# Human-Augment-Analytics/vectordb-retrieval

Measured on AMD Instinct MI355X. Metric: QPS @ recall@10 (SIFT1M-shaped, 10k-query batch, k=10), higher is better.
Workload: dtype i8 MFMA scan (i32 accumulate) + exact integer / f64 refine

## Files before the change

vectordb-retrieval_amd/csrc/common.hpp:

```cpp
#pragma once
#include <hip/hip_runtime.h>
#include <hip/hip_fp16.h>
#include <stdint.h>

#include <stdexcept>
#include <string>

namespace vdb {

constexpr int kTileRows = 32;
constexpr int kSpanRows = 512;
constexpr int kBinRows = 256;
constexpr int kTilesPerSpan = 16;
constexpr int kTileRows16 = 16;
constexpr int kSpanRows16 = 1024;
constexpr int kTilesPerSpan16 = 64;
constexpr int kIvfTilesPerSpan = 8;
constexpr int kIvfSpanRows = kIvfTilesPerSpan * kTileRows;
constexpr int kStageTiles = 4;
constexpr int kMaxKSteps = 8;
constexpr float kPadBias = 1.0e38f;

constexpr int kStatShards = 32;
constexpr int kStatStride = 16;
__device__ __forceinline__ void stat_add(unsigned long long *counters, long long q, int idx, unsigned long long v) {
    atomicAdd(&counters[(size_t)(q & (kStatShards - 1)) * kStatStride + idx], v);
}
constexpr size_t kSmallBytes = 64 + (size_t)kStatShards * kStatStride * 8;
constexpr size_t kInfoOffset = 16;

struct IndexStats {
    unsigned absmax_bits;
    unsigned maxnorm2_bits;
    int nonfinite;
    int not_integer;
    int not_fp16_exact;
    int not_u8;
    int not_s8;
    int pad[1];
};

struct QueryBatchInfo {
    unsigned absmax_bits;
    int not_integer;
    int not_fp16_exact;
    int nonfinite;
    float sq;
    float cs;
    float bscale;
    int force_fallback;
    int not_u8, not_s8;
    int i8_mode;
    unsigned done_blocks;
};
static_assert(sizeof(QueryBatchInfo) + 16 <= 64, "QueryBatchInfo must fit the first 64 bytes of ws.small");

__host__ __device__ inline int group_rows_of(int i8_mode) { return (i8_mode & 4) ? 8 : 4; }
__host__ __device__ inline int cand_row_offset(unsigned packed_bits, int i8_mode) {
    return (int)(packed_bits & 0x3Fu) * group_rows_of(i8_mode);
}
constexpr int kI8Offset = 1 << 24;
constexpr int kI8PadBias = 30000000;
constexpr unsigned kI8Inf = 0x7f800000u;

struct Range {
    int64_t row0;
    int32_t count;
    int32_t pad;
};

__host__ __device__ inline uint64_t sortable_u64(double v) {
    uint64_t u = *reinterpret_cast<uint64_t *>(&v);
    return (u & 0x8000000000000000ull) ? ~u : (u | 0x8000000000000000ull);
}
__host__ __device__ inline double unsortable_f64(uint64_t k) {
    uint64_t u = (k & 0x8000000000000000ull) ? (k & 0x7fffffffffffffffull) : ~k;
    return *reinterpret_cast<double *>(&u);
}
__host__ __device__ inline unsigned sortable_u32(float v) {
    unsigned u = *reinterpret_cast<unsigned *>(&v);
    return (u & 0x80000000u) ? ~u : (u | 0x80000000u);
}
__host__ __device__ inline float unsortable_f32(unsigned k) {
    unsigned u = (k & 0x80000000u) ? (k & 0x7fffffffu) : ~k;
    return *reinterpret_cast<float *>(&u);
}

struct Error : public std::runtime_error {
    int code;
    Error(int c, const std::string &m) : std::runtime_error(m), code(c) {}
};

#define VDB_HIP(expr)                                                                              \
    do {                                                                                           \
        hipError_t e__ = (expr);                                                                   \
        if (e__ != hipSuccess)                                                                     \
            throw ::vdb::Error(3, std::string(#expr) + " failed: " + hipGetErrorString(e__));      \
    } while (0)

}
```

vectordb-retrieval_amd/csrc/refine.hpp:

```cpp
#pragma once
#include "common.hpp"
#include "topk.hpp"

namespace vdb {

struct Sq8Rows {
    const unsigned char *codes = nullptr;
    const int32_t *list = nullptr;
    const float *cent = nullptr;
    const float *vmin = nullptr;
    const float *vdiff = nullptr;
};

__device__ __forceinline__ float sq8_decode(unsigned code, float c, float vmin, float vdiff) {
    return c + (vmin + (((float)code + 0.5f) / 255.0f) * vdiff);
}

struct PqRows {
    const unsigned char *codes = nullptr;
    const float *cb = nullptr;
    int M = 0, dsub = 0;
};

struct RefineCommon {
// ... 80 lines not shown
    const unsigned *cw = reinterpret_cast<const unsigned *>(s.codes + (size_t)row * D4);
    const float4 *cv = reinterpret_cast<const float4 *>(s.cent + (size_t)s.list[row] * D4);
    const float4 *mv = reinterpret_cast<const float4 *>(s.vmin);
    const float4 *dv = reinterpret_cast<const float4 *>(s.vdiff);
    const float4 *qv = reinterpret_cast<const float4 *>(q);
    double acc = 0.0;
#pragma unroll 4
    for (int i = 0; i < D4 / 4; ++i) {
        const unsigned w = cw[i];
        const float4 c = cv[i], m = mv[i], d = dv[i], b = qv[i];
        const double x0 = (double)sq8_decode(w & 0xffu, c.x, m.x, d.x);
        const double x1 = (double)sq8_decode((w >> 8) & 0xffu, c.y, m.y, d.y);
        const double x2 = (double)sq8_decode((w >> 16) & 0xffu, c.z, m.z, d.z);
        const double x3 = (double)sq8_decode(w >> 24, c.w, m.w, d.w);
        if (metric == 0) {
            double t;
            t = x0 - (double)b.x; acc = fma(t, t, acc);
            t = x1 - (double)b.y; acc = fma(t, t, acc);
            t = x2 - (double)b.z; acc = fma(t, t, acc);
            t = x3 - (double)b.w; acc = fma(t, t, acc);
        } else {
            acc = fma((double)b.x, x0, acc);
            acc = fma((double)b.y, x1, acc);
            acc = fma((double)b.z, x2, acc);
            acc = fma((double)b.w, x3, acc);
        }
    }
    return sortable_u64(metric == 0 ? acc : -acc);
}

__device__ __forceinline__ uint64_t pq_key(const PqRows &p, int64_t row, const float *__restrict__ q, int D4, int metric) {
    const unsigned char *cr = p.codes + (size_t)row * p.M;
    double acc = 0.0;
    int d = 0;
    for (int m = 0; m < p.M; ++m) {
        const float *cv = p.cb + ((size_t)m * 256 + cr[m]) * p.dsub;
        for (int j = 0; j < p.dsub; ++j, ++d) {
            const double x = (double)cv[j];
            if (metric == 0) {
                const double t = x - (double)q[d];
                acc = fma(t, t, acc);
            } else {
                acc = fma((double)q[d], x, acc);
            }
        }
    }
    for (; d < D4; ++d) {
        if (metric == 0) {
            const double t = 0.0 - (double)q[d];
            acc = fma(t, t, acc);
        } else {
            acc = fma((double)q[d], 0.0, acc);
        }
    }
    return sortable_u64(metric == 0 ? acc : -acc);
}

template <int U = 16>
__device__ __forceinline__ uint64_t row_key(const RefineCommon &c, int64_t row, const float *__restrict__ q) {
    if (c.X) return exact_key<U>(c.X + (size_t)row * c.D4, q, c.D4, c.metric);
    if (c.sq8.codes) return sq8_key(c.sq8, row, q, c.D4, c.metric);
    if (c.pq.codes) return pq_key(c.pq, row, q, c.D4, c.metric);
    return exact_key_i8<U>(c.X8 + (size_t)row * c.x8_pitch, c.cx, q, c.D4, c.metric);
}

template <int QB>
__device__ __forceinline__ void exact_keys(const float *__restrict__ x, const float *const (&q)[QB], int D4, int metric,
                                           uint64_t (&out)[QB]) {
    const float4 *xv = reinterpret_cast<const float4 *>(x);
    double acc[QB];
#pragma unroll
    for (int j = 0; j < QB; ++j) acc[j] = 0.0;
#pragma unroll 4
    for (int i = 0; i < D4 / 4; ++i) {
        const float4 a = xv[i];
#pragma unroll
        for (int j = 0; j < QB; ++j) {
            const float4 b = reinterpret_cast<const float4 *>(q[j])[i];
            if (metric == 0) {
                double t;
                t = (double)a.x - (double)b.x; acc[j] = fma(t, t, acc[j]);
                t = (double)a.y - (double)b.y; acc[j] = fma(t, t, acc[j]);
                t = (double)a.z - (double)b.z; acc[j] = fma(t, t, acc[j]);
                t = (double)a.w - (double)b.w; acc[j] = fma(t, t, acc[j]);
            } else {
                acc[j] = fma((double)b.x, (double)a.x, acc[j]);
                acc[j] = fma((double)b.y, (double)a.y, acc[j]);
                acc[j] = fma((double)b.z, (double)a.z, acc[j]);
                acc[j] = fma((double)b.w, (double)a.w, acc[j]);
            }
        }
    }
#pragma unroll
    for (int j = 0; j < QB; ++j) out[j] = sortable_u64(metric == 0 ? acc[j] : -acc[j]);
}

template <int KPL, int U = 16>
__device__ __forceinline__ void scan_rows(WaveTopK<KPL> &tk, const RefineCommon &c, const float *qptr, int64_t row0,
                                          int64_t row1) {
    const int lane = threadIdx.x & 63;
    if (row1 > c.N) row1 = c.N;
    for (int64_t base = row0; base < row1; base += 64) {
        const int64_t row = base + lane;
        const bool valid = row < row1;
        uint64_t key = ~0ull;
        if (valid) key = row_key<U>(c, row, qptr);
        tk.offer(key, c.idmap ? (valid ? c.idmap[row] : -1) : c.id_base + row, valid);
    }
}

template <int KPL>
__device__ __forceinline__ void write_topk(const WaveTopK<KPL> &tk, int metric, float *D, int64_t *I, double *pk,
                                           int64_t *pi) {
    const int lane = threadIdx.x & 63;
#pragma unroll
    for (int e = 0; e < KPL; ++e) {
        const int s = e * 64 + lane;
        if (s < tk.k) {
            const bool have = s < tk.n;
            const double kv = have ? unsortable_f64(tk.key[e]) : __builtin_inf();
            if (D) {
                float d;
                if (have)
                    d = (float)(metric == 0 ? kv : -kv);
                else
                    d = (metric == 0) ? 3.402823466e+38f : -3.402823466e+38f;
                D[s] = d;
                I[s] = have ? tk.id[e] : -1;
            } else {
                pk[s] = kv;
                pi[s] = have ? tk.id[e] : -1;
            }
        }
    }
}

struct RefineListArgs {
    RefineCommon c;
    int64_t nq;
    const int32_t *cand_rows;
    const int32_t *rescan_rows;
    const int32_t *counts;
    const int32_t *fallback;
    int cand_cap;
    int rescan_cap;
    float *D;
    int64_t *I;
    double *pkeys;
    int64_t *pids;
    int group_shift = -1;
    int f16_shift = 2;
};

template <int KPL, int W>
__device__ __forceinline__ void refine_list_dot8(const RefineListArgs &a, int64_t q, int ncand, int nres, int gshift,
                                                 WaveTopK<KPL> &tk) {
    const int lane = threadIdx.x & 63;
    const RefineCommon &c = a.c;
    const int mode = c.info->i8_mode;
    const int cq = (mode & 3) == 1 ? 127 : -1;
    int qb[W];
    const int *q8 = reinterpret_cast<const int *>(c.Q8 + (size_t)q * c.x8_pitch);
#pragma unroll
    for (int w = 0; w < W; ++w) qb[w] = __builtin_amdgcn_readfirstlane(q8[w]);
    int sq = 0, sqq = 0;
    const float *qf = c.Q + (size_t)q * c.D4;
    for (int d = lane; d < c.D4; d += 64) {
        const int v = (int)qf[d];
        sq += v;
        sqq += v * v;
    }
#pragma unroll
    for (int o = 32; o > 0; o >>= 1) {
        sq += __shfl_xor(sq, o);
        sqq += __shfl_xor(sqq, o);
    }
    const long long cxq = (long long)c.cx * sq - (long long)c.D * c.cx * cq;
    auto key_of = [&](int64_t row) -> uint64_t {
        const refine_int4 *xr = reinterpret_cast<const refine_int4 *>(c.X8 + (size_t)row * c.x8_pitch);
        const int2 st = reinterpret_cast<const int2 *>(c.rowstat)[row];
        int dot = 0;
#pragma unroll
        for (int i = 0; i < W / 4; ++i) {
            const refine_int4 w = xr[i];
            dot = __builtin_amdgcn_sdot4(w.x, qb[4 * i], dot, false);
            dot = __builtin_amdgcn_sdot4(w.y, qb[4 * i + 1], dot, false);
            dot = __builtin_amdgcn_sdot4(w.z, qb[4 * i + 2], dot, false);
            dot = __builtin_amdgcn_sdot4(w.w, qb[4 * i + 3], dot, false);
        }
        const long long xq = -(long long)dot + (long long)cq * st.y + cxq;
        return c.metric == 0 ? sortable_u64((double)((long long)st.x - 2 * xq + sqq)) : sortable_u64(-(double)xq);
    };
    const int32_t *cr = a.cand_rows + (size_t)q * a.cand_cap;
    for (int base = 0; base < (ncand << gshift); base += 64) {
        const int i = base + lane;
        bool valid = i < (ncand << gshift);
        const int64_t row = valid ? (int64_t)cr[i >> gshift] + (i & ((1 << gshift) - 1)) : 0;
        valid = valid && row < c.N;
        const uint64_t key = valid ? key_of(row) : ~0ull;
        tk.offer(key, c.idmap ? (valid ? c.idmap[row] : -1) : c.id_base + row, valid);
    }
    const int32_t *rr = a.rescan_rows + (size_t)q * a.rescan_cap * 2;
    for (int r = 0; r < nres; ++r) {
        const int64_t row0 = rr[2 * r];
        int64_t row1 = rr[2 * r + 1];
        if (row1 > c.N) row1 = c.N;
        for (int64_t base = row0; base < row1; base += 64) {
            const int64_t row = base + lane;
            const bool valid = row < row1;
            const uint64_t key = valid ? key_of(row) : ~0ull;
            tk.offer(key, c.idmap ? (valid ? c.idmap[row] : -1) : c.id_base + row, valid);
        }
    }
}

template <int KPL>
__device__ __forceinline__ void refine_list_body(const RefineListArgs &a, unsigned block) {
    const int lane = threadIdx.x & 63;
    const int64_t q = __builtin_amdgcn_readfirstlane((int)(block * 4 + (threadIdx.x >> 6)));
    if (q >= a.nq) return;
    if (a.fallback[q]) return;
    const float *qptr = a.c.Q + (size_t)q * a.c.D4;
    WaveTopK<KPL> tk;
    tk.init(a.c.k);
    int ncand = a.counts[2 * q];
    int nres = a.counts[2 * q + 1];
    ncand = ncand < a.cand_cap ? ncand : a.cand_cap;
    nres = nres < a.rescan_cap ? nres : a.rescan_cap;
    const int32_t *cr = a.cand_rows + (size_t)q * a.cand_cap;
    const int mode = a.c.info != nullptr ? a.c.info->i8_mode : 0;
    const int gshift = a.group_shift >= 0 ? a.group_shift : mode ? ((mode & 4) ? 3 : 2) : a.f16_shift;
    if (mode != 0 && a.c.X8 != nullptr) {
        if (a.c.x8_pitch == 64) refine_list_dot8<KPL, 16>(a, q, ncand, nres, gshift, tk);
        else refine_list_dot8<KPL, 32>(a, q, ncand, nres, gshift, tk);
    } else {
        for (int base = 0; base < (ncand << gshift); base += 64) {
            const int i = base + lane;
            bool valid = i < (ncand << gshift);
            int64_t row = valid ? (int64_t)cr[i >> gshift] + (i & ((1 << gshift) - 1)) : 0;
            valid = valid && row < a.c.N;
            uint64_t key = ~0ull;
            if (valid) key = row_key(a.c, row, qptr);
            tk.offer(key, a.c.idmap ? (valid ? a.c.idmap[row] : -1) : a.c.id_base + row, valid);
        }
        const int32_t *rr = a.rescan_rows + (size_t)q * a.rescan_cap * 2;
        for (int r = 0; r < nres; ++r) scan_rows<KPL>(tk, a.c, qptr, rr[2 * r], rr[2 * r + 1]);
    }
    const size_t o = (size_t)q * a.c.k;
    write_topk<KPL>(tk, a.c.metric, a.D ? a.D + o : nullptr, a.I ? a.I + o : nullptr, a.pkeys ? a.pkeys + o : nullptr,
                    a.pids ? a.pids + o : nullptr);
}

struct RefineFallbackArgs {
    RefineCommon c;
    const int32_t *fb_list;
    const int32_t *fb_count;
    int max_split;
    int64_t cap_units;
    double *pkeys;
    int64_t *pids;
    int32_t *done;
    float *D;
    int64_t *I;
    double *okeys;
    int64_t *oids;
};

template <int KPL>
__device__ __forceinline__ void refine_fallback_body(const RefineFallbackArgs &a, unsigned block, unsigned nblocks) {
    const int64_t count = *a.fb_count;
    if (count <= 0) return;
    const int lane = threadIdx.x & 63;
    const int64_t waves = (int64_t)nblocks * 4;
    const int64_t wave0 = __builtin_amdgcn_readfirstlane((int)(block * 4 + (threadIdx.x >> 6)));
    int64_t S = waves / count;
    if (S > a.max_split) S = a.max_split;
    if (S > a.cap_units / count) S = a.cap_units / count;
    if (S < 1) S = 1;
    const int64_t rows_per_split = ((a.c.N + S - 1) / S + 63) / 64 * 64;
    for (int64_t u = wave0; u < count * S; u += waves) {
        const int64_t f = u / S;
        const int split = (int)(u - f * S);
        const int64_t q = a.fb_list[f];
        WaveTopK<KPL> tk;
        tk.init(a.c.k);
        scan_rows<KPL, 4>(tk, a.c, a.c.Q + (size_t)q * a.c.D4, (int64_t)split * rows_per_split, (int64_t)(split + 1) * rows_per_split);
        const size_t oq = (size_t)q * a.c.k;
        if (S == 1) {
            if (a.D) write_topk<KPL>(tk, a.c.metric, a.D + oq, a.I + oq, nullptr, nullptr);
            else write_topk<KPL>(tk, a.c.metric, nullptr, nullptr, a.okeys + oq, a.oids + oq);
            continue;
        }
        write_topk<KPL>(tk, a.c.metric, nullptr, nullptr, a.pkeys + (size_t)u * a.c.k, a.pids + (size_t)u * a.c.k);
        __threadfence();
        int last = 0;
        if (lane == 0) last = atomicAdd(&a.done[f], 1) == (int)S - 1;
        last = __builtin_amdgcn_readfirstlane(last);
        if (!last) continue;
        __threadfence();
        if (lane == 0) a.done[f] = 0;
        tk.init(a.c.k);
        const int total = (int)S * a.c.k;
        const size_t o0 = (size_t)f * S * a.c.k;
        for (int base = 0; base < total; base += 64) {
            const int i = base + lane;
            bool valid = i < total;
            uint64_t key = ~0ull;
            int64_t id = -1;
            if (valid) {
                id = __builtin_nontemporal_load(a.pids + o0 + i);
                key = sortable_u64(__builtin_nontemporal_load(a.pkeys + o0 + i));
                valid = id >= 0;
            }
            tk.offer(key, id, valid);
        }
        if (a.D) write_topk<KPL>(tk, a.c.metric, a.D + oq, a.I + oq, nullptr, nullptr);
        else write_topk<KPL>(tk, a.c.metric, nullptr, nullptr, a.okeys + oq, a.oids + oq);
    }
}

template <int KPL>
__global__ __launch_bounds__(256, (KPL == 1 ? 6 : KPL == 2 ? 5 : 1)) void refine_tail_kernel(RefineListArgs la, RefineFallbackArgs fa, unsigned fb_blocks) {
    if (blockIdx.x < fb_blocks) refine_fallback_body<KPL>(fa, blockIdx.x, fb_blocks);
    else refine_list_body<KPL>(la, blockIdx.x - fb_blocks);
}

struct RerankArgs {
    RefineCommon c;
    int64_t nq;
    const int64_t *cand;
    int ncand;
    float *D;
    int64_t *I;
    double *pkeys = nullptr;
    int64_t *pids = nullptr;
    const int64_t *segs = nullptr;
    int nseg = 0;
};

template <int KPL>
__global__ __launch_bounds__(256) void rerank_kernel(RerankArgs a) {
    const int lane = threadIdx.x & 63;
    const int64_t q = __builtin_amdgcn_readfirstlane((int)(blockIdx.x * 4 + (threadIdx.x >> 6)));
    if (q >= a.nq) return;
    const float *qptr = a.c.Q + (size_t)q * a.c.D4;
    WaveTopK<KPL> tk;
    tk.init(a.c.k);
    const int64_t *cr = a.cand + (size_t)q * a.ncand;
    for (int base = 0; base < a.ncand; base += 64) {
        const int i = base + lane;
        bool valid = i < a.ncand;
        const int64_t id = valid ? cr[i] : -1;
        int64_t row = id - a.c.id_base;
        if (a.segs) {
            row = -1;
            for (int j = 0; j < a.nseg; ++j) {
                const int64_t id0 = a.segs[3 * j];
                if (id >= id0 && id < id0 + a.segs[3 * j + 2]) row = a.segs[3 * j + 1] + (id - id0);
            }
        }
        valid = valid && id >= 0 && row >= 0 && row < a.c.N;
        uint64_t key = ~0ull;
        if (valid) key = row_key(a.c, row, qptr);
        tk.offer(key, id, valid);
    }
    const size_t o = (size_t)q * a.c.k;
    write_topk<KPL>(tk, a.c.metric, a.D ? a.D + o : nullptr, a.I ? a.I + o : nullptr, a.pkeys ? a.pkeys + o : nullptr,
                    a.pids ? a.pids + o : nullptr);
}

struct RefineFullArgs {
    RefineCommon c;
    const int32_t *qlist;
    const int32_t *count_ptr;
    int64_t count;
    int S;
    int64_t rows_per_split;
    float *D;
    int64_t *I;
    double *pkeys;
    int64_t *pids;
};

template <int KPL>
__global__ __launch_bounds__(256) void refine_full_kernel(RefineFullArgs a) {
    const int64_t waves_total = (int64_t)gridDim.x * 4;
    const int64_t wave0 = __builtin_amdgcn_readfirstlane((int)(blockIdx.x * 4 + (threadIdx.x >> 6)));
    const int64_t count = a.count_ptr ? (int64_t)*a.count_ptr : a.count;
    const int64_t units = count * a.S;
    for (int64_t u = wave0; u < units; u += waves_total) {
        const int64_t slot = u / a.S;
        const int split = (int)(u - slot * a.S);
        const int64_t q = a.qlist ? (int64_t)a.qlist[slot] : slot;
        const float *qptr = a.c.Q + (size_t)q * a.c.D4;
        WaveTopK<KPL> tk;
        tk.init(a.c.k);
        const int64_t r0 = (int64_t)split * a.rows_per_split;
        scan_rows<KPL>(tk, a.c, qptr, r0, r0 + a.rows_per_split);
        if (a.D) {
            const size_t o = (size_t)q * a.c.k;
            write_topk<KPL>(tk, a.c.metric, a.D + o, a.I + o, nullptr, nullptr);
        } else {
            const size_t o = (size_t)u * a.c.k;
            write_topk<KPL>(tk, a.c.metric, nullptr, nullptr, a.pkeys + o, a.pids + o);
        }
    }
}

template <int KPL, int QB, bool PQ = false>
__global__ __launch_bounds__(256) void refine_full_blocked_kernel(RefineFullArgs a) {
    const int lane = threadIdx.x & 63;
    const int64_t waves_total = (int64_t)gridDim.x * 4;
    const int64_t wave0 = __builtin_amdgcn_readfirstlane((int)(blockIdx.x * 4 + (threadIdx.x >> 6)));
    const int64_t count = a.count_ptr ? (int64_t)*a.count_ptr : a.count;
    const int64_t groups = (count + QB - 1) / QB;
    const int64_t units = groups * a.S;
    for (int64_t u = wave0; u < units; u += waves_total) {
        const int64_t grp = u / a.S;
        const int split = (int)(u - grp * a.S);
        int64_t slot[QB], q[QB];
        const float *qptr[QB];
        WaveTopK<KPL> tk[QB];
#pragma unroll
        for (int j = 0; j < QB; ++j) {
            slot[j] = grp * QB + j;
            const int64_t sj = slot[j] < count ? slot[j] : count - 1;
            q[j] = a.qlist ? (int64_t)a.qlist[sj] : sj;
            qptr[j] = a.c.Q + (size_t)q[j] * a.c.D4;
            tk[j].init(a.c.k);
        }
        const int64_t r0 = (int64_t)split * a.rows_per_split;
        int64_t r1 = r0 + a.rows_per_split;
        if (r1 > a.c.N) r1 = a.c.N;
        for (int64_t base = r0; base < r1; base += 64) {
            const int64_t row = base + lane;
            const bool valid = row < r1;
            uint64_t key[QB];
#pragma unroll
            for (int j = 0; j < QB; ++j) key[j] = ~0ull;
            if (valid) {
                if (PQ) {
#pragma unroll
                    for (int j = 0; j < QB; ++j) key[j] = pq_key(a.c.pq, row, qptr[j], a.c.D4, a.c.metric);
                } else if (a.c.X) {
                    exact_keys<QB>(a.c.X + (size_t)row * a.c.D4, qptr, a.c.D4, a.c.metric, key);
                } else {
#pragma unroll
                    for (int j = 0; j < QB; ++j)
                        key[j] = exact_key_i8<4>(a.c.X8 + (size_t)row * a.c.x8_pitch, a.c.cx, qptr[j], a.c.D4, a.c.metric);
                }
            }
            const int64_t id = a.c.idmap ? (valid ? a.c.idmap[row] : -1) : a.c.id_base + row;
#pragma unroll
            for (int j = 0; j < QB; ++j) tk[j].offer(key[j], id, valid);
        }
#pragma unroll
        for (int j = 0; j < QB; ++j) {
            if (slot[j] < count) {
                if (a.D) {
                    const size_t o = (size_t)q[j] * a.c.k;
                    write_topk<KPL>(tk[j], a.c.metric, a.D + o, a.I + o, nullptr, nullptr);
                } else {
                    const size_t o = (size_t)(slot[j] * a.S + split) * a.c.k;
                    write_topk<KPL>(tk[j], a.c.metric, nullptr, nullptr, a.pkeys + o, a.pids + o);
                }
            }
        }
    }
}

struct MergeArgs {
    const double *pkeys;
    const int64_t *pids;
    int64_t part_stride;
    int64_t slot_stride;
    int nparts;
    int k;
// ... 53 lines not shown
```

vectordb-retrieval_amd/csrc/scan.hpp:

```cpp
#pragma once
#include "common.hpp"
#include "prep.hpp"

namespace vdb {

typedef float float16v __attribute__((ext_vector_type(16)));

struct ScanArgs {
    const half8 *panels;
    const float *bias;
    const half8 *qpanels;
    const QueryBatchInfo *info;
    float *bin_m1;
    float *bin_m2;
    float *bin_m3;
    float *sb_m1;
    float *sb_m2;
    int32_t *sb_span;
    int64_t nspans;
    int spans_per_chunk;
    int chunk_rem;
    int nchunks;
    int chunk0;
    int nqtiles;
// ... 371 lines not shown
}

template <int VPL>
__global__ __launch_bounds__(256) void select_kernel(SelectArgs a) {
    const int lane = threadIdx.x & 63;
    const int64_t q = __builtin_amdgcn_readfirstlane((int)(blockIdx.x * 4 + (threadIdx.x >> 6)));
    if (q >= a.nq) return;
    const int dbps = a.direct_rows ? kBinRows / a.direct_rows : 0;
    const int nsb = a.direct_rows ? (int)a.nspans * a.groups * dbps : a.nchunks * a.groups;
    unsigned v[VPL];
    float sv[VPL];
#pragma unroll
    for (int e = 0; e < VPL; ++e) sv[e] = a.sb_m1[(size_t)min(e * 64 + lane, nsb - 1) * a.Qpad + q];
#pragma unroll
    for (int e = 0; e < VPL; ++e) asm volatile("" : "+v"(sv[e]));
#pragma unroll
    for (int e = 0; e < VPL; ++e) v[e] = (e * 64 + lane < nsb) ? sortable_u32(sv[e]) : 0xFFFFFFFFu;
    unsigned ans = 0;
    if (VPL >= 4 && a.k <= 64) {
        unsigned lo0 = 0xFFFFFFFFu, lo1 = 0xFFFFFFFFu;
#pragma unroll
        for (int e = 0; e < VPL; ++e) {
            const unsigned x = v[e];
            lo1 = min(lo1, max(lo0, x));
            lo0 = min(lo0, x);
        }
        for (int bit = 31; bit >= 0; --bit) {
            const unsigned trial = ans | ((1u << bit) - 1u);
            const int cnt = __popcll(__ballot(lo0 <= trial)) + __popcll(__ballot(lo1 <= trial));
            if (cnt < a.k) ans |= (1u << bit);
        }
    } else {
        for (int bit = 31; bit >= 0; --bit) {
            const unsigned trial = ans | ((1u << bit) - 1u);
            int cnt = 0;
#pragma unroll
            for (int e = 0; e < VPL; ++e) cnt += __popcll(__ballot(v[e] <= trial));
            if (cnt < a.k) ans |= (1u << bit);
        }
    }
    const float tau = unsortable_f32(ans);
    const int i8_mode = a.info->i8_mode;
    const float that = select_threshold(tau, a.eps[q], i8_mode);
    const int gmode = i8_mode ? i8_mode : a.f16_gmode;
    const bool force_fb = a.info->force_fallback || !(that < 0.9e38f) || nsb < a.k;

    int ncand = 0, nres = 0;
    int32_t *cr = a.cand_rows + (size_t)q * a.cand_cap;
    int32_t *rr = a.rescan_rows + (size_t)q * a.rescan_cap * 2;
    const unsigned long long lt_mask = (1ull << lane) - 1ull;

    if (!force_fb) {
        float sm2v[VPL];
        int spanv[VPL];
#pragma unroll
        for (int e = 0; e < VPL; ++e) sm2v[e] = a.sb_m2[(size_t)min(e * 64 + lane, nsb - 1) * a.Qpad + q];
#pragma unroll
        for (int e = 0; e < VPL; ++e) spanv[e] = a.direct_rows ? 0 : a.sb_span[(size_t)min(e * 64 + lane, nsb - 1) * a.Qpad + q];
#pragma unroll
        for (int e = 0; e < VPL; ++e) asm volatile("" : "+v"(sm2v[e]), "+v"(spanv[e]));
#pragma unroll
        for (int e = 0; e < VPL; ++e) {
            const int s = e * 64 + lane;
            const bool in = s < nsb;
            const float m1 = in ? unsortable_f32(v[e]) : __builtin_inff();
            const bool active = in && (m1 <= that);
            const float sm2 = active ? sm2v[e] : __builtin_inff();
            const int sspan = active ? spanv[e] : 0;
            if (a.direct_rows) {
                const int row0 = (s / dbps) * kBinRows + (s % dbps) * a.direct_rows;
                const bool single = active && !(sm2 <= that), deep = active && !single;
                const unsigned long long smask = __ballot(single), rmask = __ballot(deep);
                if (single) {
                    const int pos = ncand + __popcll(smask & lt_mask);
                    if (pos < a.cand_cap) cr[pos] = row0 + cand_row_offset(__float_as_uint(m1), gmode);
                }
                if (deep) {
                    const int pos = nres + __popcll(rmask & lt_mask);
                    if (pos < a.rescan_cap) {
                        rr[2 * pos] = row0;
                        rr[2 * pos + 1] = row0 + a.direct_rows;
                    }
                }
                ncand += __popcll(smask);
                nres += __popcll(rmask);
                continue;
            }
            const bool single = active && !(sm2 <= that);
            const unsigned long long smask = __ballot(single);
            if (single) {
                const int pos = ncand + __popcll(smask & lt_mask);
                const int hh = s % a.groups;
                const int row = (sspan * a.groups + hh) * kBinRows + cand_row_offset(__float_as_uint(m1), gmode);
                if (pos < a.cand_cap) cr[pos] = row;
            }
            ncand += __popcll(smask);
            unsigned long long dmask = __ballot(active && !single);
            while (dmask) {
                const int src = __ffsll(dmask) - 1;
                dmask &= dmask - 1;
                const int sb = e * 64 + src;
                const int chunk = sb / a.groups, hh = sb % a.groups;
                const int64_t sp0 = chunk_span0(chunk, a.spans_per_chunk, a.chunk_rem);
                int64_t sp1 = chunk_span0(chunk + 1, a.spans_per_chunk, a.chunk_rem);
                if (sp1 > a.nspans) sp1 = a.nspans;
                for (int64_t base = sp0; base < sp1; base += 64) {
                    const int64_t sp = base + lane;
                    bool act = false, resc = false;
                    float bm1 = 0.f;
                    if (sp < sp1) {
                        const size_t o = (size_t)(sp * a.groups + hh) * a.Qpad + q;
                        bm1 = a.bin_m1[o];
                        if (bm1 <= that) {
                            act = true;
                            resc = a.bin_m2[o] <= that;
                        }
                    }
                    const bool cand = act && !resc;
                    const unsigned long long cm = __ballot(cand), rm = __ballot(resc);
                    if (cand) {
                        const int pos = ncand + __popcll(cm & lt_mask);
                        if (pos < a.cand_cap)
                            cr[pos] = (int)((sp * a.groups + hh) * kBinRows + cand_row_offset(__float_as_uint(bm1), gmode));
                    }
                    if (resc) {
                        const int pos = nres + __popcll(rm & lt_mask);
                        if (pos < a.rescan_cap) {
                            rr[2 * pos] = (int)((sp * a.groups + hh) * kBinRows);
                            rr[2 * pos + 1] = rr[2 * pos] + kBinRows;
                        }
                    }
                    ncand += __popcll(cm);
                    nres += __popcll(rm);
                }
            }
        }
    }
    const bool fb = force_fb || ncand > a.cand_cap || nres > a.rescan_cap;
    if (lane == 0) {
        a.counts[2 * q] = fb ? 0 : ncand;
        a.counts[2 * q + 1] = fb ? 0 : nres;
        a.fallback[q] = fb ? 1 : 0;
        if (fb) {
            const int pos = atomicAdd(a.fb_count, 1);
            a.fb_list[pos] = (int)q;
            stat_add(a.stat_counters, q, 2, 1ull);
        } else {
            stat_add(a.stat_counters, q, 0, (unsigned long long)ncand);
            stat_add(a.stat_counters, q, 1, (unsigned long long)nres);
        }
    }
}

template <int V, int LPQ>
__global__ __launch_bounds__(256, 1) void select_kernel_v2(SelectArgs a) {
    constexpr int QPW = 64 / LPQ;
    constexpr int kDeepCap = 48;
    __shared__ int s_cnt[4][QPW][3];
    __shared__ int s_deep[4][QPW][kDeepCap];
    const int lane = threadIdx.x & 63, wave = threadIdx.x >> 6;
    const int qi = lane / LPQ, part = lane % LPQ;
    const int64_t q = ((int64_t)blockIdx.x * 4 + wave) * QPW + qi;
    const bool qvalid = q < a.nq;
    const int nsb = a.nchunks * a.groups;
    if (part < 3) s_cnt[wave][qi][part] = 0;
    unsigned v[V];
    float sv[V];
#pragma unroll
    for (int e = 0; e < V; ++e) sv[e] = a.sb_m1[(size_t)min(e * LPQ + part, nsb - 1) * a.Qpad + q];
#pragma unroll
    for (int e = 0; e < V; ++e) asm volatile("" : "+v"(sv[e]));
#pragma unroll
    for (int e = 0; e < V; ++e) v[e] = (e * LPQ + part < nsb) ? sortable_u32(sv[e]) : 0xFFFFFFFFu;
    unsigned ans = 0;
    for (int bit = 31; bit >= 0; --bit) {
        const unsigned trial = ans | ((1u << bit) - 1u);
        int cnt = 0;
#pragma unroll
        for (int e = 0; e < V; ++e) cnt += (v[e] <= trial) ? 1 : 0;
#pragma unroll
        for (int o = 1; o < LPQ; o <<= 1) cnt += __shfl_xor(cnt, o);
        if (cnt < a.k) ans |= (1u << bit);
    }
    const float tau = unsortable_f32(ans);
    const int i8_mode = a.info->i8_mode;
    const float that = select_threshold(tau, qvalid ? a.eps[q] : 0.f, i8_mode);
    const int gmode = i8_mode ? i8_mode : a.f16_gmode;
    const bool force_fb = a.info->force_fallback || !(that < 0.9e38f) || nsb < a.k;
    __syncthreads();
    int *cnt_c = &s_cnt[wave][qi][0], *cnt_r = &s_cnt[wave][qi][1], *cnt_d = &s_cnt[wave][qi][2];
    int *deep = &s_deep[wave][qi][0];
    bool deep_overflow = false;
    if (qvalid && !force_fb) {
        int32_t *cr = a.cand_rows + (size_t)q * a.cand_cap;
        float sm2v[V];
        int spanv[V];
#pragma unroll
        for (int e = 0; e < V; ++e) {
            const int s = e * LPQ + part;
            const bool act = (s < nsb) && (unsortable_f32(v[e]) <= that);
            sm2v[e] = act ? a.sb_m2[(size_t)s * a.Qpad + q] : __builtin_inff();
            spanv[e] = act ? a.sb_span[(size_t)s * a.Qpad + q] : 0;
        }
#pragma unroll
        for (int e = 0; e < V; ++e) {
            const int s = e * LPQ + part;
            if (s >= nsb) continue;
            const float m1 = unsortable_f32(v[e]);
            if (!(m1 <= that)) continue;
            const int hh = s % a.groups;
            if (!(sm2v[e] <= that)) {
                const int pos = atomicAdd(cnt_c, 1);
                if (pos < a.cand_cap)
                    cr[pos] = (spanv[e] * a.groups + hh) * kBinRows + cand_row_offset(__float_as_uint(m1), gmode);
            } else {
                const int pos = atomicAdd(cnt_d, 1);
                if (pos < kDeepCap) deep[pos] = s;
            }
        }
    }
    __syncthreads();
    {
        const int nd_q = (qvalid && !force_fb) ? *cnt_d : 0;
        int nd_max = nd_q;
#pragma unroll
        for (int o = 1; o < 64; o <<= 1) nd_max = max(nd_max, __shfl_xor(nd_max, o));
        if (nd_q > kDeepCap) deep_overflow = true;
        int32_t *cr = a.cand_rows + (size_t)q * a.cand_cap;
        int32_t *rr = a.rescan_rows + (size_t)q * a.rescan_cap * 2;
        for (int d = 0; d < nd_max && d < kDeepCap; ++d) {
            if (d >= nd_q) continue;
            const int s = deep[d];
            const int chunk = s / a.groups, hh = s % a.groups;
            const int64_t sp0 = chunk_span0(chunk, a.spans_per_chunk, a.chunk_rem);
            int64_t sp1 = chunk_span0(chunk + 1, a.spans_per_chunk, a.chunk_rem);
            if (sp1 > a.nspans) sp1 = a.nspans;
            for (int64_t sp = sp0 + part; sp < sp1; sp += LPQ) {
                const size_t o = (size_t)(sp * a.groups + hh) * a.Qpad + q;
                const float bm1 = a.bin_m1[o];
                if (!(bm1 <= that)) continue;
                if (a.bin_m2[o] <= that) {
                    const int pos = atomicAdd(cnt_r, 1);
                    if (pos < a.rescan_cap) {
                        rr[2 * pos] = (int)((sp * a.groups + hh) * kBinRows);
                        rr[2 * pos + 1] = rr[2 * pos] + kBinRows;
                    }
                } else {
                    const int pos = atomicAdd(cnt_c, 1);
                    if (pos < a.cand_cap)
                        cr[pos] = (int)((sp * a.groups + hh) * kBinRows + cand_row_offset(__float_as_uint(bm1), gmode));
                }
            }
        }
    }
    __syncthreads();
    if (qvalid && part == 0) {
        const int ncand = *cnt_c, nres = *cnt_r;
        const bool fb = force_fb || deep_overflow || ncand > a.cand_cap || nres > a.rescan_cap;
        a.counts[2 * q] = fb ? 0 : ncand;
        a.counts[2 * q + 1] = fb ? 0 : nres;
        a.fallback[q] = fb ? 1 : 0;
        if (fb) {
            const int pos = atomicAdd(a.fb_count, 1);
            a.fb_list[pos] = (int)q;
            stat_add(a.stat_counters, q, 2, 1ull);
        } else {
            stat_add(a.stat_counters, q, 0, (unsigned long long)ncand);
            stat_add(a.stat_counters, q, 1, (unsigned long long)nres);
        }
    }
}

}
```

vectordb-retrieval_amd/csrc/topk.hpp:

```cpp
#pragma once
#include "common.hpp"

namespace vdb {

__device__ __forceinline__ bool pair_less(uint64_t ka, int64_t ia, uint64_t kb, int64_t ib) {
    return (ka < kb) || (ka == kb && ia < ib);
}

__device__ __forceinline__ uint64_t bcast_u64(uint64_t v, int src_lane) {
    unsigned lo = __builtin_amdgcn_readlane((unsigned)v, src_lane);
    unsigned hi = __builtin_amdgcn_readlane((unsigned)(v >> 32), src_lane);
    return ((uint64_t)hi << 32) | lo;
}

template <int KPL>
struct WaveTopK {
    static constexpr int kBatchMin = 12;
    uint64_t key[KPL];
    int64_t id[KPL];
    int n;
    int k;
    uint64_t thr_key;
    int64_t thr_id;

    __device__ __forceinline__ void init(int k_) {
        k = k_;
        n = 0;
        thr_key = ~0ull;
        thr_id = INT64_MAX;
#pragma unroll
        for (int e = 0; e < KPL; ++e) {
            key[e] = ~0ull;
            id[e] = -1;
        }
    }

    __device__ __forceinline__ bool beats_threshold(uint64_t nk, int64_t nid) const {
        return n < k || pair_less(nk, nid, thr_key, thr_id);
    }

    __device__ __forceinline__ void insert_uniform(uint64_t nk, int64_t nid) {
        const int lane = threadIdx.x & 63;
        int pos = 0;
#pragma unroll
        for (int e = 0; e < KPL; ++e) {
            const int s = e * 64 + lane;
            const bool lt = (s < n) && pair_less(key[e], id[e], nk, nid);
            pos += __popcll(__ballot(lt));
        }
#pragma unroll
        for (int e = KPL - 1; e >= 0; --e) {
            uint64_t upk = __shfl_up(key[e], 1);
            int64_t upi = __shfl_up(id[e], 1);
            if (e > 0) {
                const uint64_t pk = bcast_u64(key[e - 1], 63);
                const int64_t pi = (int64_t)bcast_u64((uint64_t)id[e - 1], 63);
                if (lane == 0) {
                    upk = pk;
                    upi = pi;
                }
            }
            const int s = e * 64 + lane;
            if (s > pos) {
                key[e] = upk;
                id[e] = upi;
            } else if (s == pos) {
                key[e] = nk;
                id[e] = nid;
            }
        }
        if (n < k) ++n;
        if (n == k) {
            const int ts = k - 1;
#pragma unroll
            for (int e = 0; e < KPL; ++e) {
                if (e == (ts >> 6)) {
                    thr_key = bcast_u64(key[e], ts & 63);
                    thr_id = (int64_t)bcast_u64((uint64_t)id[e], ts & 63);
                }
            }
        }
    }

    __device__ __forceinline__ static void cex_lane(uint64_t &k_, int64_t &i_, int j, bool keep_min) {
        const uint64_t ok = __shfl_xor(k_, j);
        const int64_t oi = __shfl_xor(i_, j);
        const bool other_less = pair_less(ok, oi, k_, i_);
        if (other_less == keep_min) {
            k_ = ok;
            i_ = oi;
        }
    }

    __device__ __forceinline__ void merge_batch(uint64_t bk, int64_t bi, int cnt) {
        const int lane = threadIdx.x & 63;
#pragma unroll
        for (int k2 = 2; k2 <= 64; k2 <<= 1) {
            const bool asc = (lane & k2) == 0;
#pragma unroll
            for (int j = k2 >> 1; j > 0; j >>= 1) cex_lane(bk, bi, j, ((lane & j) == 0) == asc);
        }
        bk = __shfl(bk, 63 - lane);
        bi = __shfl(bi, 63 - lane);
#pragma unroll
        for (int e = 0; e < KPL; ++e)
            if (e * 64 + lane >= n) {
                key[e] = ~0ull;
                id[e] = INT64_MAX;
            }
        if (pair_less(bk, bi, key[KPL - 1], id[KPL - 1])) {
            key[KPL - 1] = bk;
            id[KPL - 1] = bi;
        }
#pragma unroll
        for (int re = KPL >> 1; re > 0; re >>= 1) {
#pragma unroll
            for (int e = 0; e < KPL; ++e) {
                if ((e & re) == 0) {
                    const int o = e + re;
                    if (pair_less(key[o], id[o], key[e], id[e])) {
                        const uint64_t tk_ = key[e];
                        const int64_t ti_ = id[e];
                        key[e] = key[o];
                        id[e] = id[o];
                        key[o] = tk_;
                        id[o] = ti_;
                    }
                }
            }
        }
#pragma unroll
        for (int j = 32; j > 0; j >>= 1) {
#pragma unroll
            for (int e = 0; e < KPL; ++e) cex_lane(key[e], id[e], j, (lane & j) == 0);
        }
        n = (n + cnt < k) ? n + cnt : k;
#pragma unroll
        for (int e = 0; e < KPL; ++e)
            if (e * 64 + lane >= n) {
                key[e] = ~0ull;
                id[e] = -1;
            }
        if (n == k) {
            const int ts = k - 1;
#pragma unroll
            for (int e = 0; e < KPL; ++e) {
                if (e == (ts >> 6)) {
                    thr_key = bcast_u64(key[e], ts & 63);
                    thr_id = (int64_t)bcast_u64((uint64_t)id[e], ts & 63);
                }
            }
        }
    }

    __device__ __forceinline__ void offer(uint64_t nk, int64_t nid, bool valid) {
        const bool want = valid && beats_threshold(nk, nid);
        uint64_t mask = __ballot(want);
        const int cnt = __popcll(mask);
        if (cnt >= kBatchMin) {
            merge_batch(want ? nk : ~0ull, want ? nid : INT64_MAX, cnt);
            return;
        }
        while (mask) {
            const int src = __ffsll((unsigned long long)mask) - 1;
            mask &= mask - 1;
            const uint64_t bk = bcast_u64(nk, src);
            const int64_t bi = (int64_t)bcast_u64((uint64_t)nid, src);
            if (beats_threshold(bk, bi)) insert_uniform(bk, bi);
        }
    }
};

}
```

Baseline: 11.46 million.

## Add LDS rank-based top-k for k<=64 refine and DPP wave reductions

Replaces the register-resident bitonic WaveTopK in the KPL==1 refine tail path with an LDS-buffered rank-selection top-k. Candidates that beat the threshold are appended to shared memory and periodically ranked by all-pairs counting. When there is no idmap, the score and row are packed into a single 64-bit key. Query i8 vectors move to LDS instead of scalar registers, and the shuffle-based reductions in refine and select become DPP/permlane16 sums. This cuts shuffle and bitonic-merge overhead but adds LDS traffic and per-block shared memory, which may lower occupancy.

Result: no change. 11.50 million, median of 6 (+0.4%).

```diff
diff --git a/vectordb-retrieval_amd/csrc/common.hpp b/vectordb-retrieval_amd/csrc/common.hpp
--- a/vectordb-retrieval_amd/csrc/common.hpp
+++ b/vectordb-retrieval_amd/csrc/common.hpp
@@ -20,6 +20,20 @@
 constexpr int kStageTiles = 4;
 constexpr int kMaxKSteps = 8;
 constexpr float kPadBias = 1.0e38f;
+
+__device__ __forceinline__ int dpp_row_sum(int v) {
+    v += __builtin_amdgcn_update_dpp(0, v, 0x121, 0xf, 0xf, false);
+    v += __builtin_amdgcn_update_dpp(0, v, 0x122, 0xf, 0xf, false);
+    v += __builtin_amdgcn_update_dpp(0, v, 0x124, 0xf, 0xf, false);
+    v += __builtin_amdgcn_update_dpp(0, v, 0x128, 0xf, 0xf, false);
+    return v;
+}
+
+__device__ __forceinline__ int wave_sum(int v) {
+    v = dpp_row_sum(v);
+    return __builtin_amdgcn_readlane(v, 0) + __builtin_amdgcn_readlane(v, 16) + __builtin_amdgcn_readlane(v, 32) +
+           __builtin_amdgcn_readlane(v, 48);
+}
 
 constexpr int kStatShards = 32;
 constexpr int kStatStride = 16;
diff --git a/vectordb-retrieval_amd/csrc/refine.hpp b/vectordb-retrieval_amd/csrc/refine.hpp
--- a/vectordb-retrieval_amd/csrc/refine.hpp
+++ b/vectordb-retrieval_amd/csrc/refine.hpp
@@ -256,17 +256,68 @@
     int f16_shift = 2;
 };
 
-template <int KPL, int W>
+template <class F>
+__device__ __forceinline__ void for_list_rows(const RefineListArgs &a, int64_t q, int ncand, int nres, int gshift, F &&f) {
+    const int lane = threadIdx.x & 63;
+    const int32_t *cr = a.cand_rows + (size_t)q * a.cand_cap;
+    const int32_t *rr = a.rescan_rows + (size_t)q * a.rescan_cap * 2;
+    for (int seg = 0; seg <= nres; ++seg) {
+        const bool cand = seg == 0;
+        const int64_t row0 = cand ? 0 : rr[2 * seg - 2];
+        const int64_t row1 = cand ? 0 : (rr[2 * seg - 1] < a.c.N ? rr[2 * seg - 1] : a.c.N);
+        const int cnt = cand ? (ncand << gshift) : (int)(row1 - row0);
+        for (int base = 0; base < cnt; base += 64) {
+            const int i = base + lane;
+            bool valid = i < cnt;
+            int64_t row = row0 + i;
+            if (cand) {
+                row = valid ? (int64_t)cr[i >> gshift] + (i & ((1 << gshift) - 1)) : 0;
+                valid = valid && row < a.c.N;
+            }
+            f(valid ? row : 0, valid);
+        }
+    }
+}
+
+template <int W>
+struct QRowScalar {
+    int v[W];
+    __device__ __forceinline__ explicit QRowScalar(const int *q8) {
+#pragma unroll
+        for (int w = 0; w < W; ++w) v[w] = __builtin_amdgcn_readfirstlane(q8[w]);
+    }
+    __device__ __forceinline__ refine_int4 quad(int i) const {
+        refine_int4 r;
+        r.x = v[4 * i];
+        r.y = v[4 * i + 1];
+        r.z = v[4 * i + 2];
+        r.w = v[4 * i + 3];
+        return r;
+    }
+};
+
+template <int W>
+struct QRowLds {
+    const refine_int4 *p;
+    __device__ __forceinline__ QRowLds(const int *q8, int *lds) : p(reinterpret_cast<const refine_int4 *>(lds)) {
+        const int lane = threadIdx.x & 63;
+        if (lane < W) lds[lane] = q8[lane];
+        wave_lds_fence();
+    }
+    __device__ __forceinline__ refine_int4 quad(int i) const { return p[i]; }
+};
+
+__device__ __forceinline__ uint64_t dot8_key(int metric, long long s) {
+    return metric == 0 ? sortable_u64((double)s) : sortable_u64(-(double)s);
+}
+
+template <int W, class QRow, class Offer>
 __device__ __forceinline__ void refine_list_dot8(const RefineListArgs &a, int64_t q, int ncand, int nres, int gshift,
-                                                 WaveTopK<KPL> &tk) {
+                                                 const QRow &qrow, Offer &&offer) {
     const int lane = threadIdx.x & 63;
     const RefineCommon &c = a.c;
     const int mode = c.info->i8_mode;
     const int cq = (mode & 3) == 1 ? 127 : -1;
-    int qb[W];
-    const int *q8 = reinterpret_cast<const int *>(c.Q8 + (size_t)q * c.x8_pitch);
-#pragma unroll
-    for (int w = 0; w < W; ++w) qb[w] = __builtin_amdgcn_readfirstlane(q8[w]);
     int sq = 0, sqq = 0;
     const float *qf = c.Q + (size_t)q * c.D4;
     for (int d = lane; d < c.D4; d += 64) {
@@ -274,84 +325,119 @@
         sq += v;
         sqq += v * v;
     }
-#pragma unroll
-    for (int o = 32; o > 0; o >>= 1) {
-        sq += __shfl_xor(sq, o);
-        sqq += __shfl_xor(sqq, o);
-    }
+    sq = wave_sum(sq);
+    sqq = wave_sum(sqq);
     const long long cxq = (long long)c.cx * sq - (long long)c.D * c.cx * cq;
-    auto key_of = [&](int64_t row) -> uint64_t {
-        const refine_int4 *xr = reinterpret_cast<const refine_int4 *>(c.X8 + (size_t)row * c.x8_pitch);
-        const int2 st = reinterpret_cast<const int2 *>(c.rowstat)[row];
-        int dot = 0;
-#pragma unroll
-        for (int i = 0; i < W / 4; ++i) {
-            const refine_int4 w = xr[i];
-            dot = __builtin_amdgcn_sdot4(w.x, qb[4 * i], dot, false);
-            dot = __builtin_amdgcn_sdot4(w.y, qb[4 * i + 1], dot, false);
-            dot = __builtin_amdgcn_sdot4(w.z, qb[4 * i + 2], dot, false);
-            dot = __builtin_amdgcn_sdot4(w.w, qb[4 * i + 3], dot, false);
-        }
-        const long long xq = -(long long)dot + (long long)cq * st.y + cxq;
-        return c.metric == 0 ? sortable_u64((double)((long long)st.x - 2 * xq + sqq)) : sortable_u64(-(double)xq);
-    };
-    const int32_t *cr = a.cand_rows + (size_t)q * a.cand_cap;
-    for (int base = 0; base < (ncand << gshift); base += 64) {
-        const int i = base + lane;
-        bool valid = i < (ncand << gshift);
-        const int64_t row = valid ? (int64_t)cr[i >> gshift] + (i & ((1 << gshift) - 1)) : 0;
-        valid = valid && row < c.N;
-        const uint64_t key = valid ? key_of(row) : ~0ull;
-        tk.offer(key, c.idmap ? (valid ? c.idmap[row] : -1) : c.id_base + row, valid);
-    }
-    const int32_t *rr = a.rescan_rows + (size_t)q * a.rescan_cap * 2;
-    for (int r = 0; r < nres; ++r) {
-        const int64_t row0 = rr[2 * r];
-        int64_t row1 = rr[2 * r + 1];
-        if (row1 > c.N) row1 = c.N;
-        for (int64_t base = row0; base < row1; base += 64) {
-            const int64_t row = base + lane;
-            const bool valid = row < row1;
-            const uint64_t key = valid ? key_of(row) : ~0ull;
-            tk.offer(key, c.idmap ? (valid ? c.idmap[row] : -1) : c.id_base + row, valid);
-        }
-    }
-}
-
-template <int KPL>
-__device__ __forceinline__ void refine_list_body(const RefineListArgs &a, unsigned block) {
-    const int lane = threadIdx.x & 63;
+    for_list_rows(a, q, ncand, nres, gshift, [&](int64_t row, bool valid) {
+        long long s = 0;
+        if (valid) {
+            const refine_int4 *xr = reinterpret_cast<const refine_int4 *>(c.X8 + (size_t)row * c.x8_pitch);
+            const int2 st = reinterpret_cast<const int2 *>(c.rowstat)[row];
+            int dot = 0;
+#pragma unroll
+            for (int i = 0; i < W / 4; ++i) {
+                const refine_int4 w = xr[i];
+                const refine_int4 b = qrow.quad(i);
+                dot = __builtin_amdgcn_sdot4(w.x, b.x, dot, false);
+                dot = __builtin_amdgcn_sdot4(w.y, b.y, dot, false);
+                dot = __builtin_amdgcn_sdot4(w.z, b.z, dot, false);
+                dot = __builtin_amdgcn_sdot4(w.w, b.w, dot, false);
+            }
+            const long long xq = -(long long)dot + (long long)cq * st.y + cxq;
+            s = c.metric == 0 ? (long long)st.x - 2 * xq + sqq : xq;
+        }
+        offer(s, row, valid);
+    });
+}
+
+constexpr int kRefineLdsWords = RankTopK<false>::kRegionBytes / 8 + 16;
+
+template <int W>
+__device__ __forceinline__ void refine_list_dot8_rank(const RefineListArgs &a, int64_t q, int ncand, int nres, int gshift,
+                                                      uint64_t *lds, WaveTopK<1> &tk) {
+    const RefineCommon &c = a.c;
+    const QRowLds<W> qrow(reinterpret_cast<const int *>(c.Q8 + (size_t)q * c.x8_pitch),
+                          reinterpret_cast<int *>(lds + RankTopK<false>::kRegionBytes / 8));
+    if (c.idmap == nullptr) {
+        RankTopK<true> rk;
+        rk.init(lds, c.k);
+        refine_list_dot8<W>(a, q, ncand, nres, gshift, qrow, [&](long long s, int64_t row, bool valid) {
+            const long long ord = (c.metric == 0 ? s : -s) + (1ll << 31);
+            rk.offer(((uint64_t)(uint32_t)ord << 32) | (uint32_t)row, 0, valid);
+        });
+        uint64_t w;
+        int64_t unused;
+        rk.finish(w, unused);
+        const long long ord = (long long)(w >> 32) - (1ll << 31);
+        tk.n = rk.n;
+        if ((int)(threadIdx.x & 63) < rk.n) {
+            tk.key[0] = dot8_key(c.metric, c.metric == 0 ? ord : -ord);
+            tk.id[0] = c.id_base + (int64_t)(uint32_t)w;
+        }
+    } else {
+        RankTopK<false> rk;
+        rk.init(lds, c.k);
+        refine_list_dot8<W>(a, q, ncand, nres, gshift, qrow, [&](long long s, int64_t row, bool valid) {
+            rk.offer(dot8_key(c.metric, s), valid ? c.idmap[row] : -1, valid);
+        });
+        rk.finish(tk.key[0], tk.id[0]);
+        tk.n = rk.n;
+    }
+}
+
+template <int KPL, bool RANK = false>
+__device__ __forceinline__ void refine_list_body(const RefineListArgs &a, unsigned block, uint64_t *lds = nullptr) {
+    static_assert(!RANK || KPL == 1, "RankTopK holds at most 64 entries");
     const int64_t q = __builtin_amdgcn_readfirstlane((int)(block * 4 + (threadIdx.x >> 6)));
     if (q >= a.nq) return;
     if (a.fallback[q]) return;
-    const float *qptr = a.c.Q + (size_t)q * a.c.D4;
+    const RefineCommon &c = a.c;
+    const float *qptr = c.Q + (size_t)q * c.D4;
     WaveTopK<KPL> tk;
-    tk.init(a.c.k);
+    tk.init(c.k);
     int ncand = a.counts[2 * q];
     int nres = a.counts[2 * q + 1];
     ncand = ncand < a.cand_cap ? ncand : a.cand_cap;
     nres = nres < a.rescan_cap ? nres : a.rescan_cap;
-    const int32_t *cr = a.cand_rows + (size_t)q * a.cand_cap;
-    const int mode = a.c.info != nullptr ? a.c.info->i8_mode : 0;
+    const int mode = c.info != nullptr ? c.info->i8_mode : 0;
     const int gshift = a.group_shift >= 0 ? a.group_shift : mode ? ((mode & 4) ? 3 : 2) : a.f16_shift;
-    if (mode != 0 && a.c.X8 != nullptr) {
-        if (a.c.x8_pitch == 64) refine_list_dot8<KPL, 16>(a, q, ncand, nres, gshift, tk);
-        else refine_list_dot8<KPL, 32>(a, q, ncand, nres, gshift, tk);
+    const bool dot8 = mode != 0 && c.X8 != nullptr;
+    if constexpr (RANK) {
+        if (dot8) {
+            if (c.x8_pitch == 64) refine_list_dot8_rank<16>(a, q, ncand, nres, gshift, lds, tk);
+            else refine_list_dot8_rank<32>(a, q, ncand, nres, gshift, lds, tk);
+        } else {
+            RankTopK<false> rk;
+            rk.init(lds, c.k);
+            for_list_rows(a, q, ncand, nres, gshift, [&](int64_t row, bool valid) {
+                uint64_t key = ~0ull;
+                if (valid) key = row_key(c, row, qptr);
+                rk.offer(key, c.idmap ? (valid ? c.idmap[row] : -1) : c.id_base + row, valid);
+            });
+            rk.finish(tk.key[0], tk.id[0]);
+            tk.n = rk.n;
+        }
     } else {
-        for (int base = 0; base < (ncand << gshift); base += 64) {
-            const int i = base + lane;
-            bool valid = i < (ncand << gshift);
-            int64_t row = valid ? (int64_t)cr[i >> gshift] + (i & ((1 << gshift) - 1)) : 0;
-            valid = valid && row < a.c.N;
-            uint64_t key = ~0ull;
-            if (valid) key = row_key(a.c, row, qptr);
-            tk.offer(key, a.c.idmap ? (valid ? a.c.idmap[row] : -1) : a.c.id_base + row, valid);
-        }
-        const int32_t *rr = a.rescan_rows + (size_t)q * a.rescan_cap * 2;
-        for (int r = 0; r < nres; ++r) scan_rows<KPL>(tk, a.c, qptr, rr[2 * r], rr[2 * r + 1]);
-    }
-    const size_t o = (size_t)q * a.c.k;
-    write_topk<KPL>(tk, a.c.metric, a.D ? a.D + o : nullptr, a.I ? a.I + o : nullptr, a.pkeys ? a.pkeys + o : nullptr,
+        const auto offer_row = [&](uint64_t key, int64_t row, bool valid) {
+            tk.offer(key, c.idmap ? (valid ? c.idmap[row] : -1) : c.id_base + row, valid);
+        };
+        if (dot8) {
+            const int *q8 = reinterpret_cast<const int *>(c.Q8 + (size_t)q * c.x8_pitch);
+            const auto offer_score = [&](long long s, int64_t row, bool valid) {
+                offer_row(valid ? dot8_key(c.metric, s) : ~0ull, row, valid);
+            };
+            if (c.x8_pitch == 64) refine_list_dot8<16>(a, q, ncand, nres, gshift, QRowScalar<16>(q8), offer_score);
+            else refine_list_dot8<32>(a, q, ncand, nres, gshift, QRowScalar<32>(q8), offer_score);
+        } else {
+            for_list_rows(a, q, ncand, nres, gshift, [&](int64_t row, bool valid) {
+                uint64_t key = ~0ull;
+                if (valid) key = row_key(c, row, qptr);
+                offer_row(key, row, valid);
+            });
+        }
+    }
+    const size_t o = (size_t)q * c.k;
+    write_topk<KPL>(tk, c.metric, a.D ? a.D + o : nullptr, a.I ? a.I + o : nullptr, a.pkeys ? a.pkeys + o : nullptr,
                     a.pids ? a.pids + o : nullptr);
 }
 
@@ -425,8 +511,14 @@
 
 template <int KPL>
 __global__ __launch_bounds__(256, (KPL == 1 ? 6 : KPL == 2 ? 5 : 1)) void refine_tail_kernel(RefineListArgs la, RefineFallbackArgs fa, unsigned fb_blocks) {
-    if (blockIdx.x < fb_blocks) refine_fallback_body<KPL>(fa, blockIdx.x, fb_blocks);
-    else refine_list_body<KPL>(la, blockIdx.x - fb_blocks);
+    if constexpr (KPL == 1) {
+        __shared__ __attribute__((aligned(16))) uint64_t s_list[4][kRefineLdsWords];
+        if (blockIdx.x < fb_blocks) refine_fallback_body<KPL>(fa, blockIdx.x, fb_blocks);
+        else refine_list_body<1, true>(la, blockIdx.x - fb_blocks, s_list[__builtin_amdgcn_readfirstlane((int)(threadIdx.x >> 6))]);
+    } else {
+        if (blockIdx.x < fb_blocks) refine_fallback_body<KPL>(fa, blockIdx.x, fb_blocks);
+        else refine_list_body<KPL>(la, blockIdx.x - fb_blocks);
+    }
 }
 
 struct RerankArgs {
diff --git a/vectordb-retrieval_amd/csrc/scan.hpp b/vectordb-retrieval_amd/csrc/scan.hpp
--- a/vectordb-retrieval_amd/csrc/scan.hpp
+++ b/vectordb-retrieval_amd/csrc/scan.hpp
@@ -547,6 +547,17 @@
     }
 }
 
+template <int LPQ>
+__device__ __forceinline__ int query_lanes_sum(int v) {
+    static_assert(LPQ == 16 || LPQ == 32, "a query owns one or two DPP rows");
+    v = dpp_row_sum(v);
+    if (LPQ == 32) {
+        const auto sw = __builtin_amdgcn_permlane16_swap((unsigned)v, (unsigned)v, false, false);
+        v = (int)(sw[0] + sw[1]);
+    }
+    return v;
+}
+
 template <int V, int LPQ>
 __global__ __launch_bounds__(256, 1) void select_kernel_v2(SelectArgs a) {
     constexpr int QPW = 64 / LPQ;
@@ -567,21 +578,22 @@
     for (int e = 0; e < V; ++e) asm volatile("" : "+v"(sv[e]));
 #pragma unroll
     for (int e = 0; e < V; ++e) v[e] = (e * LPQ + part < nsb) ? sortable_u32(sv[e]) : 0xFFFFFFFFu;
+    const int i8_mode = a.info->i8_mode;
+    const int info_fb = a.info->force_fallback;
+    const float eps_q = qvalid ? a.eps[q] : 0.f;
     unsigned ans = 0;
     for (int bit = 31; bit >= 0; --bit) {
         const unsigned trial = ans | ((1u << bit) - 1u);
         int cnt = 0;
 #pragma unroll
         for (int e = 0; e < V; ++e) cnt += (v[e] <= trial) ? 1 : 0;
-#pragma unroll
-        for (int o = 1; o < LPQ; o <<= 1) cnt += __shfl_xor(cnt, o);
+        cnt = query_lanes_sum<LPQ>(cnt);
         if (cnt < a.k) ans |= (1u << bit);
     }
     const float tau = unsortable_f32(ans);
-    const int i8_mode = a.info->i8_mode;
-    const float that = select_threshold(tau, qvalid ? a.eps[q] : 0.f, i8_mode);
+    const float that = select_threshold(tau, eps_q, i8_mode);
     const int gmode = i8_mode ? i8_mode : a.f16_gmode;
-    const bool force_fb = a.info->force_fallback || !(that < 0.9e38f) || nsb < a.k;
+    const bool force_fb = info_fb || !(that < 0.9e38f) || nsb < a.k;
     __syncthreads();
     int *cnt_c = &s_cnt[wave][qi][0], *cnt_r = &s_cnt[wave][qi][1], *cnt_d = &s_cnt[wave][qi][2];
     int *deep = &s_deep[wave][qi][0];
diff --git a/vectordb-retrieval_amd/csrc/topk.hpp b/vectordb-retrieval_amd/csrc/topk.hpp
--- a/vectordb-retrieval_amd/csrc/topk.hpp
+++ b/vectordb-retrieval_amd/csrc/topk.hpp
@@ -171,4 +171,124 @@
     }
 };
 
-}
+typedef unsigned long long topk_u64x2 __attribute__((ext_vector_type(2)));
+
+__device__ __forceinline__ void wave_lds_fence() {
+    __builtin_amdgcn_fence(__ATOMIC_ACQ_REL, "wavefront");
+    __builtin_amdgcn_wave_barrier();
+}
+
+template <bool ONE>
+struct RankTopK {
+    static constexpr int kCap = 256;
+    static constexpr int kRegionBytes = kCap * (ONE ? 8 : 16);
+    static constexpr int kUnroll = ONE ? 8 : 4;
+    uint64_t *r;
+    int n;
+    int fill;
+    int k;
+    uint64_t thr_key;
+    int64_t thr_id;
+
+    __device__ __forceinline__ static bool less(uint64_t ka, int64_t ia, uint64_t kb, int64_t ib) {
+        return ONE ? ka < kb : pair_less(ka, ia, kb, ib);
+    }
+    __device__ __forceinline__ void put(int s, uint64_t kk, int64_t ii) {
+        if (ONE) {
+            r[s] = kk;
+        } else {
+            topk_u64x2 v;
+            v.x = kk;
+            v.y = (uint64_t)ii;
+            reinterpret_cast<topk_u64x2 *>(r)[s] = v;
+        }
+    }
+    __device__ __forceinline__ void get(int s, uint64_t &kk, int64_t &ii) const {
+        if (ONE) {
+            kk = r[s];
+            ii = 0;
+        } else {
+            const topk_u64x2 v = reinterpret_cast<const topk_u64x2 *>(r)[s];
+            kk = v.x;
+            ii = (int64_t)v.y;
+        }
+    }
+
+    __device__ __forceinline__ void init(uint64_t *region, int k_) {
+        r = region;
+        k = k_;
+        n = fill = 0;
+        thr_key = ~0ull;
+        thr_id = INT64_MAX;
+    }
+
+    template <int P>
+    __device__ __forceinline__ void rank_round(int T) {
+        const int lane = threadIdx.x & 63;
+        uint64_t ok[P];
+        int64_t oi[P];
+        int c[P];
+#pragma unroll
+        for (int p = 0; p < P; ++p) {
+            ok[p] = ~0ull;
+            oi[p] = INT64_MAX;
+            c[p] = 0;
+            if (lane + 64 * p < T) get(lane + 64 * p, ok[p], oi[p]);
+        }
+        const int TU = (T + kUnroll - 1) & ~(kUnroll - 1);
+        if (lane < TU - T) put(T + lane, ~0ull, INT64_MAX);
+        wave_lds_fence();
+        for (int j = 0; j < TU; j += kUnroll) {
+            uint64_t ek[kUnroll];
+            int64_t ei[kUnroll];
+#pragma unroll
+            for (int u = 0; u < kUnroll; ++u) get(j + u, ek[u], ei[u]);
+#pragma unroll
+            for (int u = 0; u < kUnroll; ++u)
+#pragma unroll
+                for (int p = 0; p < P; ++p) c[p] += less(ek[u], ei[u], ok[p], oi[p]) ? 1 : 0;
+        }
+        wave_lds_fence();
+#pragma unroll
+        for (int p = 0; p < P; ++p)
+            if (lane + 64 * p < T && c[p] < k) put(c[p], ok[p], oi[p]);
+        wave_lds_fence();
+    }
+
+    __device__ __forceinline__ void flush() {
+        const int T = fill;
+        if (T <= 64) rank_round<1>(T);
+        else if (T <= 128) rank_round<2>(T);
+        else rank_round<4>(T);
+        n = T < k ? T : k;
+        fill = n;
+        if (n == k) {
+            uint64_t tk_;
+            int64_t ti_;
+            get(k - 1, tk_, ti_);
+            thr_key = bcast_u64(tk_, 0);
+            thr_id = (int64_t)bcast_u64((uint64_t)ti_, 0);
+        }
+    }
+
+    __device__ __forceinline__ void offer(uint64_t nk, int64_t nid, bool valid) {
+        const bool want = valid && (n < k || less(nk, nid, thr_key, thr_id));
+        const uint64_t mask = __ballot(want);
+        const int cnt = __popcll(mask);
+        if (cnt == 0) return;
+        const int pos = fill + (int)__builtin_amdgcn_mbcnt_hi((unsigned)(mask >> 32), __builtin_amdgcn_mbcnt_lo((unsigned)mask, 0u));
+        if (want) put(pos, nk, nid);
+        fill += cnt;
+        if ((n < k && fill >= k) || fill > kCap - 64) flush();
+    }
+
+    __device__ __forceinline__ void finish(uint64_t &kk, int64_t &ii) {
+        if (fill > n) flush();
+        const int lane = threadIdx.x & 63;
+        kk = ~0ull;
+        ii = -1;
+        if (lane < n) get(lane, kk, ii);
+    }
+};
+
+}
```
